# ebartrum/lightning_gan_zoo

Measured on AMD Instinct MI355X. Metric: images/sec (G+D step) at 64x64 bs=128/GPU, higher is better.
Workload: dtype f32; 1 GPU; dc_gan synthetic 64x64 bs=128/GPU, one optimizer cycle of 2 batches (Lightning alternation + toggle), reference optimizer, fp32; key=dc_gan_bs128, global_batch=128, parallelism=dp1, images_counted=2*bs*n_gpus per step (every batch of the cycle)

## Files before the change

include/gz_ops.h:

```cpp
#ifndef GZ_OPS_H
#define GZ_OPS_H

#include <stddef.h>

#ifdef __cplusplus
extern "C" {
#endif

#ifndef __HIP__
typedef struct ihipStream_t* hipStream_t;
#endif

#define GZ_ACT_NONE 0
#define GZ_ACT_RELU 1
#define GZ_ACT_LRELU 2
#define GZ_ACT_TANH 3


long long gz_conv2d_pack_fwd_elems(int K, int C, int KH, int KW);
long long gz_conv2d_pack_dgrad_elems(int K, int C, int KH, int KW, int S);

int gz_conv2d_pack_fwd(const float* w, float* wpack, int K, int C, int KH, int KW, hipStream_t stream);
int gz_conv2d_pack_dgrad(const float* w, float* wpack, int K, int C, int KH, int KW, int S, int P,
                         hipStream_t stream);
// ... 21 lines not shown

size_t gz_conv2d_wgrad_workspace_bytes(int N, int C, int H, int W, int K, int OH, int OW, int KH, int KW);
int gz_conv2d_wgrad_fuses_bias(int N, int C, int H, int W, int K, int OH, int OW, int KH, int KW, int S, int P);
int gz_conv2d_wgrad(const float* x, const float* y, float* dw, float* dbias, float* workspace, size_t ws_bytes, int N,
                    int C, int H, int W, int K, int OH, int OW, int KH, int KW, int S, int P, hipStream_t stream);

int gz_set_cu_budget(int cu_count);
int gz_get_cu_budget(void);

int gz_conv2d_plan(int op, int N, int C, int H, int W, int K, int OH, int OW, int KH, int KW, int S, int P, char* buf,
                   int buflen);

int gz_conv2d_wgrad_partial(const float* x, const float* y, float* dw, float* workspace, size_t ws_bytes, int N, int C,
                            int H, int W, int K, int OH, int OW, int KH, int KW, int S, int P, int* nz_out,
                            long long* stride_out, hipStream_t stream);
int gz_conv2d_wgrad_act_fuses(int N, int C, int H, int W, int K, int OH, int OW, int KH, int KW, int S, int P, int act);
int gz_conv2d_wgrad_act_partial(const float* x, const float* gy, const float* fwd_out, int act, float slope,
                                float* workspace, size_t ws_bytes, int N, int C, int H, int W, int K, int OH, int OW,
                                int KH, int KW, int S, int P, int* nz_out, long long* stride_out,
                                long long* bias_offset_out, hipStream_t stream);
int gz_conv2d_dgrad_act_fuses(int N, int C, int H, int W, int K, int OH, int OW, int KH, int KW, int S, int P, int act);
int gz_conv2d_dgrad_act(const float* gy, const float* fwd_out, int act, float slope, const float* wpack, float* x, int N,
                        int C, int H, int W, int K, int OH, int OW, int KH, int KW, int S, int P, hipStream_t stream);
int gz_reduce_multi_max_jobs(void);
int gz_reduce_multi_max_sources(void);
size_t gz_reduce_multi_table_bytes(void);
int gz_reduce_multi_add(void* table_host, float* out, long long count, int beta, const float* slabs, int nz,
                        long long stride);
int gz_reduce_multi(void* table_host, hipStream_t stream);

int gz_conv2d_fwd_stats_rows(int N, int C, int H, int W, int K, int OH, int OW, int KH, int KW, int S, int P);
int gz_conv2d_fwd_stats(const float* x, const float* wpack, float* y, float* stats, int N, int C, int H, int W, int K,
                        int OH, int OW, int KH, int KW, int S, int P, hipStream_t stream);
int gz_conv2d_dgrad_stats_rows(int N, int C, int H, int W, int K, int OH, int OW, int KH, int KW, int S, int P);
int gz_conv2d_fwd_stats_ws(const float* x, const float* wpack, float* y, float* stats, float* workspace, size_t ws_bytes,
                           int N, int C, int H, int W, int K, int OH, int OW, int KH, int KW, int S, int P,
                           hipStream_t stream);
int gz_conv2d_dgrad_stats_ws(const float* y, const float* wpack, float* x, float* stats, float* workspace,
                             size_t ws_bytes, int N, int C, int H, int W, int K, int OH, int OW, int KH, int KW, int S,
                             int P, hipStream_t stream);
int gz_conv2d_dgrad_stats(const float* y, const float* wpack, float* x, float* stats, int N, int C, int H, int W, int K,
                          int OH, int OW, int KH, int KW, int S, int P, hipStream_t stream);

int gz_conv2d_tile(int op, int N, int C, int H, int W, int K, int OH, int OW, int KH, int KW, int S);

int gz_gemm(const float* a, const float* b, const float* bias, float* c, float* workspace, size_t ws_bytes, int M,
// ... 247 lines not shown
```

lightning_gan_zoo_amd/core/models/standard_networks.py:

```python
import math
from collections import OrderedDict

import torch
from torch import nn

from ... import functional as F


class _GBlock(nn.Module):

    def __init__(self, cin, cout, stride, padding):
        super().__init__()
        self.transpose_conv = nn.ConvTranspose2d(cin, cout, 4, stride, padding, bias=False)
        self.batch_norm = nn.BatchNorm2d(cout)
        self.relu = nn.ReLU()
        self.stride, self.padding = stride, padding

    def forward(self, x):
        w = self.transpose_conv.weight
        bn = self.batch_norm
        F.ready(w, bn.weight, bn.bias)
        training = bn.training or bn.running_mean is None
        stats = None
        if self.stride == 1 and self.padding == 0 and x.shape[2] == 1 and x.shape[3] == 1:
            n = x.shape[0]
            y = F.matmul(x.reshape(n, -1), w.view(w.shape[0], -1), w).view(n, w.shape[1], 4, 4)
        elif self.stride == 2 and self.padding == 1:
            if training:
                y, stats = F.conv_transpose2d_with_stats(x, w, F.K4S2P1)
            else:
                y = F.conv_transpose2d(x, w, None, F.K4S2P1)
        else:
            raise RuntimeError("unsupported transposed-convolution geometry on the HIP path")
        return F.batch_norm_act(y, bn.weight, bn.bias, bn.running_mean, bn.running_var, bn.num_batches_tracked,
                                training, bn.momentum, bn.eps, F.ACT_RELU, 0.0, stats)


class _DBlock(nn.Module):

    def __init__(self, cin, cout, norm):
        super().__init__()
        self.conv = nn.Conv2d(cin, cout, 4, 2, 1, bias=False)
        if norm == "batch_norm":
            self.batch_norm = nn.BatchNorm2d(cout)
        elif norm == "instance_norm2d":
            self.instance_norm2d = nn.InstanceNorm2d(cout, affine=True)
        else:
            self.identity = nn.Identity()
        self.leaky_relu = nn.LeakyReLU(0.2)
        self.norm = norm

    def forward(self, x, groups=1):
        slope = self.leaky_relu.negative_slope
        F.ready(*self.parameters())
        if self.norm == "batch_norm":
            bn = self.batch_norm
# ... 33 lines not shown
    supports_stacked_batches = True
    gates_parameters = True

    def __init__(self, channels_img, features_d, norm="batch_norm", img_size=64, final_sigmoid=True):
        super().__init__()
        self.norm = norm
        n_blocks = int(math.log2(img_size // 8))
        blocks = [(f"block{i}", _DBlock(features_d * 2 ** (i - 1), features_d * 2 ** i, norm))
                  for i in range(1, n_blocks + 1)]
        conv_in = nn.Conv2d(channels_img, features_d, kernel_size=4, stride=2, padding=1, bias=False)
        conv_out = nn.Conv2d(features_d * 2 ** n_blocks, 1, kernel_size=4, stride=2, padding=0, bias=False)
        tail = ("sigmoid", nn.Sigmoid()) if final_sigmoid else ("identity", nn.Identity())
        self.disc = _DiscStack(OrderedDict(
            [("conv_in", conv_in), ("leaky_relu", nn.LeakyReLU(0.2))] + blocks + [("conv_out", conv_out), tail]))

    def forward(self, x, groups=1):
        if groups > 1 and self.norm == "batch_norm" and not self.training:
            raise RuntimeError("stacked batches with their own statistics exist in training mode only")
        return self.disc(x, groups)


class _GenStack(nn.Sequential):
    def forward(self, x):
        for name, m in self.named_children():
            if name.startswith("block"):
                x = m(x)
        F.ready(self.transpose_conv_out.weight)
        return F.conv_transpose2d(x, self.transpose_conv_out.weight, None, F.K4S2P1, F.ACT_TANH, 0.0)


class Generator(nn.Module):
    gates_parameters = True

    def __init__(self, channels_noise, channels_img, features_g, img_size=64):
        super().__init__()
        n_blocks = int(math.log2(img_size / 4))
        widths = [channels_noise] + [features_g * 2 ** (n_blocks - i) for i in range(n_blocks)]
        layers = [(f"block{i + 1}", _GBlock(widths[i], widths[i + 1], 1 if i == 0 else 2, 0 if i == 0 else 1))
                  for i in range(n_blocks)]
        layers.append(("transpose_conv_out", nn.ConvTranspose2d(features_g * 2, channels_img, kernel_size=4,
                                                                stride=2, padding=1, bias=False)))
        layers.append(("tanh", nn.Tanh()))
        self.net = _GenStack(OrderedDict(layers))

    def forward(self, x):
        return self.net(x.unsqueeze(-1).unsqueeze(-1))
```

lightning_gan_zoo_amd/csrc/gz_conv.hip:

```cpp
#include <cstdio>
#include <type_traits>

#include "gz_conv_choice.h"
#include "gz_conv_direct.h"
#include "gz_igemm.h"
#include "gz_reduce.h"
#include "../../include/gz_ops.h"

namespace gz {


static TileId pick_tile2(long long M, long long N, int ny, int kdim) {
    const bool off = knobs().no_igemm2;
    if (!off && N > 32 && N <= 64 && kdim >= 256) {
        const long long t = ((M + 511) / 512) * ny;
        if (t >= 2 * cus()) return T512x64;
        if (!knobs().no_tile64 && knobs().igemm2_tile == 0 && N == 64 && ((M + 255) / 256) * ny >= cus()) return T256x64;
        return T64x64;
    }
    if (off || N < 128 || kdim < 256) return T64x64;
    const long long t128 = ((M + 255) / 256) * ((N + 127) / 128) * ny;
    const long long t256 = ((M + 255) / 256) * ((N + 255) / 256) * ny;
    const int force = knobs().igemm2_tile;
    const int cu = cus();
// ... 948 lines not shown
        return run_gemm<Cfg, MContigLoader<Cfg::BM>, MContigLoader<Cfg::BN>>(a, b, bias, c, M, N, K, lda, ldb, ldc, act, slope, st, splits, slab);
    }
    if (!ta && tb) return run_gemm<Cfg, KContigLoader<Cfg::BM>, KContigLoader<Cfg::BN>>(a, b, bias, c, M, N, K, lda, ldb, ldc, act, slope, st, splits, slab);
    return run_gemm<Cfg, MContigLoader<Cfg::BM>, KContigLoader<Cfg::BN>>(a, b, bias, c, M, N, K, lda, ldb, ldc, act, slope, st, splits, slab);
}

}

using namespace gz;

typedef Geo<4, 4, 2, 1> G4421;
typedef Geo<5, 5, 2, 2> G5522;
typedef Geo<3, 3, 1, 1> G3311;
typedef Geo<1, 1, 1, 0> G1110;

#define GZ_GEOM_DISPATCH_OR(CALL, ELSE)                                 \
    if (KH == 4 && KW == 4 && S == 2 && P == 1) return CALL(G4421);     \
    if (KH == 5 && KW == 5 && S == 2 && P == 2) return CALL(G5522);     \
    if (KH == 3 && KW == 3 && S == 1 && P == 1) return CALL(G3311);     \
    if (KH == 1 && KW == 1 && S == 1 && P == 0) return CALL(G1110);     \
    return ELSE;
#define GZ_GEOM_DISPATCH(CALL) GZ_GEOM_DISPATCH_OR(CALL, GZ_ERR_UNSUPPORTED)

extern "C" {

size_t gz_conv2d_fwd_workspace_bytes(int N, int C, int H, int W, int K, int OH, int OW, int KH, int KW, int S, int P) {
    ConvShape s{N, C, H, W, K, OH, OW};
    if (!shape_ok(s, KH, KW, S, P)) return 0;
#define CALL(G) fwd_ws_bytes<G>(s)
    GZ_GEOM_DISPATCH_OR(CALL, 0)
#undef CALL
}

size_t gz_conv2d_dgrad_workspace_bytes(int N, int C, int H, int W, int K, int OH, int OW, int KH, int KW, int S,
                                       int P) {
    ConvShape s{N, C, H, W, K, OH, OW};
    if (!shape_ok(s, KH, KW, S, P)) return 0;
#define CALL(G) dgrad_ws_bytes<G>(s)
    GZ_GEOM_DISPATCH_OR(CALL, 0)
#undef CALL
}

int gz_conv2d_fwd(const float* x, const float* wpack, const float* bias, float* y, float* workspace, size_t ws_bytes,
                  int N, int C, int H, int W, int K, int OH, int OW, int KH, int KW, int S, int P, int act,
                  float slope, hipStream_t stream) {
    gz::clear_stale_error();
// ... 84 lines not shown
}

static bool dgrad_act_direct(const ConvShape& s, int KH, int KW, int S, int P, int act) {
    return KH == 4 && KW == 4 && S == 2 && P == 1 && (act == ACT_RELU || act == ACT_LRELU) && !knobs().no_act_fuse &&
           dgrad_direct<G4421>(s) && smallc_four_pos(s);
}

int gz_conv2d_dgrad_act_fuses(int N, int C, int H, int W, int K, int OH, int OW, int KH, int KW, int S, int P, int act) {
    ConvShape s{N, C, H, W, K, OH, OW};
    return shape_ok(s, KH, KW, S, P) && dgrad_act_direct(s, KH, KW, S, P, act) ? 1 : 0;
}

int gz_conv2d_dgrad_act(const float* gy, const float* fwd_out, int act, float slope, const float* wpack, float* x, int N,
                        int C, int H, int W, int K, int OH, int OW, int KH, int KW, int S, int P, hipStream_t stream) {
    gz::clear_stale_error();
    ConvShape s{N, C, H, W, K, OH, OW};
    if (!gy || !fwd_out || !wpack || !x || !shape_ok(s, KH, KW, S, P)) return GZ_ERR_BAD_SHAPE;
    if (too_large((long long)N * C * H * W) || too_large((long long)N * K * OH * OW)) return GZ_ERR_TOO_LARGE;
    if (!dgrad_act_direct(s, KH, KW, S, P, act) || (((uintptr_t)gy | (uintptr_t)x | (uintptr_t)fwd_out | (uintptr_t)wpack) & 15))
        return GZ_ERR_UNSUPPORTED;
    const float neg = act == ACT_RELU ? 0.f : slope;
    const int ks = smallc_split((long long)N * OH * OW / 4, K);
    return run_dgrad_smallc(gy, wpack, nullptr, x, s, ACT_NONE, 0.f, stream, ks, fwd_out, neg);
}

int gz_set_cu_budget(int cu_count) {
    if (cu_count <= 0) cu_count = 256;
    if (cu_count < 64) cu_count = 64;
    if (cu_count > 256) cu_count = 256;
    gz::cu_budget_ref().store(cu_count, std::memory_order_relaxed);
    return cu_count;
}

int gz_get_cu_budget(void) { return gz::cus(); }

static int stats_wm(TileId t) { return t == T128x32 ? 4 : 2; }
static int stats_tm_rows(TileId t, long long M) {
    if (t == T256x256 || t == T256x128) return (int)((M + 255) / 256) * 2;
    if (t == T512x64) return (int)((M + 511) / 512) * 4;
    if (t == T256x64) return (int)((M + 255) / 256) * 2;
    const int bm = t == T64x64 ? 64 : 128;
    return (int)((M + bm - 1) / bm) * stats_wm(t);
}

int gz_conv2d_fwd_stats_rows(int N, int C, int H, int W, int K, int OH, int OW, int KH, int KW, int S, int P) {
    ConvShape s{N, C, H, W, K, OH, OW};
// ... 225 lines not shown
```

lightning_gan_zoo_amd/csrc/gz_conv_direct.h:

```cpp
#pragma once
#include "gz_conv_choice.h"

namespace gz {

bool smallc_four_pos(const ConvShape& s);
bool dgrad_direct5_ok(const ConvShape& s);
int smallc_split(long long M4, int K);
int run_dgrad_smallc(const float* y, const float* wp, const float* bias, float* x, const ConvShape& s, int act, float slope,
                     hipStream_t st, int ks, const float* mask = nullptr, float mask_neg = 0.f);
int run_dgrad_smallc5(const float* y, const float* wp, const float* bias, float* x, const ConvShape& s, int act, float slope,
                      hipStream_t st, int ks);

bool conv3_fewk_ok(int CI, int CO, int H, int W);
bool conv3_smallch_ok(int N, int CI, int CO, int H, int W);
int run_conv3_smallch(const float* in, const float* wp, const float* bias, float* out, int N, int CI, int CO, int H, int W,
                      int tap_major, int flip, int act, float slope, hipStream_t st, Loader ld);

bool wgrad_fewk_ok(const ConvShape& s);
bool wgrad_smallch_ok(const ConvShape& s, int KH, int KW, int S, int P);
int wgrad_smallch_blocks(const ConvShape& s);
int run_wgrad_smallch(const float* x, const float* y, float* dw, float* dbias, float* ws, size_t ws_bytes, const ConvShape& s,
                      Loader ld, hipStream_t st);

bool wgrad_k4s2p1_fewc_ok(const ConvShape& s);
int wgrad_k4s2p1_fewc_blocks(const ConvShape& s);
int run_wgrad_k4s2p1_fewc(const float* x, const float* y, const float* fwd_out, int act, float slope, float* dw, float* ws,
                          size_t ws_bytes, const ConvShape& s, hipStream_t st);

}
```

lightning_gan_zoo_amd/csrc/gz_conv_direct.hip:

```cpp
#include "gz_conv_direct.h"
#include "gz_knobs.h"
#include "gz_pack_layout.h"
#include "gz_reduce.h"
#include "../../include/gz_ops.h"

namespace gz {

template <int C>
__global__ __launch_bounds__(256) void dgrad_smallc_k4s2p1_kernel(const float* __restrict__ y,
                                                                  const float* __restrict__ wp,
                                                                  const float* __restrict__ bias,
                                                                  float* __restrict__ x, ConvShape s,
                                                                  FastDiv div_ohw, FastDiv div_ow, int act,
                                                                  float slope) {
    const int OHW = s.OH * s.OW;
    const uint32_t M = (uint32_t)s.N * OHW;
    const uint32_t m = blockIdx.x * 256u + threadIdx.x;
    const bool m_ok = m < M;
    const uint32_t n = fdiv(m, div_ohw);
    const uint32_t pix = m - n * (uint32_t)OHW;
    const int a = (int)fdiv(pix, div_ow);
    const int b = (int)(pix - (uint32_t)a * (uint32_t)s.OW);
    __amdgpu_buffer_rsrc_t rsrc = make_rsrc(y, (uint32_t)s.N * s.K * OHW * 4u);
    uint32_t voff[3][3];
// ... 31 lines not shown
                    for (int tx = 0; tx < 2; ++tx) {
                        const float yv = v[(py + 1) / 2 - ty + 1][(px + 1) / 2 - tx + 1];
                        const f32x4 w4 = *reinterpret_cast<const f32x4*>(wrow + (ty * 2 + tx) * 4);
#pragma unroll
                        for (int c = 0; c < C; ++c) acc[py][px][c] = fmaf(yv, w4[c], acc[py][px][c]);
                    }
            }
    }
    if (!m_ok) return;
#pragma unroll
    for (int c = 0; c < C; ++c) {
        const float bv = bias ? bias[c] : 0.f;
#pragma unroll
        for (int py = 0; py < 2; ++py) {
            f32x2 o;
            o.x = act_fwd(acc[py][0][c] + bv, act, slope);
            o.y = act_fwd(acc[py][1][c] + bv, act, slope);
            float* dst = x + (((long long)n * C + c) * s.H + (2 * a + py)) * s.W + 2 * b;
            *reinterpret_cast<f32x2*>(dst) = o;
        }
    }
}

template <int C, int KS, int KH = 4>
__global__ __launch_bounds__(KS > 4 ? 64 * KS : 256) void dgrad_smallc4_k4s2p1_kernel(const float* __restrict__ y,
                                                                   const float* __restrict__ wp,
                                                                   const float* __restrict__ bias,
                                                                   float* __restrict__ x, ConvShape s,
                                                                   FastDiv div_ohw4, FastDiv div_ow4, int act,
                                                                   float slope, const float* __restrict__ mask = nullptr,
                                                                   float mask_neg = 0.f) {
    constexpr int P = KH == 4 ? 1 : 2, TMAX = (KH + 1) / 2;
    __shared__ float part[KS > 1 ? KS / 2 : 1][KS > 1 ? 16 * C : 1][64];
    const int OW4 = s.OW >> 2, OHW = s.OH * s.OW;
    const uint32_t M4 = (uint32_t)s.N * s.OH * OW4;
    const int lane = threadIdx.x & 63, wave = KS > 1 ? __builtin_amdgcn_readfirstlane(threadIdx.x >> 6) : 0;
    const uint32_t m = KS > 1 ? blockIdx.x * 64u + lane : blockIdx.x * 256u + threadIdx.x;
    const bool m_ok = m < M4;
    const uint32_t n = fdiv(m, div_ohw4);
    const uint32_t pix = m - n * (uint32_t)(s.OH * OW4);
    const int a = (int)fdiv(pix, div_ow4);
    const int b = (int)(pix - (uint32_t)a * (uint32_t)OW4) * 4;
    __amdgpu_buffer_rsrc_t rsrc = make_rsrc(y, (uint32_t)s.N * s.K * OHW * 4u);
    uint32_t voff[3];
#pragma unroll
    for (int dy = 0; dy < 3; ++dy) {
        int oy = a + dy - 1;
        bool ok = m_ok && (unsigned)oy < (unsigned)s.OH;
        voff[dy] = ok ? (n * (uint32_t)(s.K * OHW) + (uint32_t)(oy * s.OW + b)) * 4u : OOB;
    }
    const bool has_l = b > 0, has_r = b + 4 < s.OW;
    float acc[4][2][2][C];
#pragma unroll
    for (int q = 0; q < 4; ++q)
#pragma unroll
        for (int i = 0; i < 2; ++i)
#pragma unroll
            for (int j = 0; j < 2; ++j)
#pragma unroll
                for (int c = 0; c < C; ++c) acc[q][i][j][c] = 0.f;
    const int kpad = round_bk(s.K);
    const long long phase_stride = KH == 4 ? (long long)s.K * 16
                                           : (long long)TMAX * TMAX * kpad * 4;
    const __amdgpu_buffer_rsrc_t rmask = make_rsrc(mask ? mask : y, (uint32_t)s.N * s.K * OHW * 4u);
    f32x4 nxt[3], mnx[3];
    if constexpr (KS > 1) {
#pragma unroll
        for (int dy = 0; dy < 3; ++dy) {
            nxt[dy] = bload4(rsrc, wave < s.K ? voff[dy] : OOB, (uint32_t)wave * (uint32_t)OHW * 4u);
            if (mask) mnx[dy] = bload4(rmask, wave < s.K ? voff[dy] : OOB, (uint32_t)wave * (uint32_t)OHW * 4u);
        }
// ... 5 lines not shown
            const bool more = ko + KS < s.K;
            const uint32_t soff = (uint32_t)(more ? ko + KS : ko) * (uint32_t)OHW * 4u;
#pragma unroll
            for (int dy = 0; dy < 3; ++dy) {
                cur[dy] = nxt[dy];
                nxt[dy] = bload4(rsrc, more ? voff[dy] : OOB, soff);
                if (mask) {
                    mcur[dy] = mnx[dy];
                    mnx[dy] = bload4(rmask, more ? voff[dy] : OOB, soff);
                }
            }
        } else {
#pragma unroll
            for (int dy = 0; dy < 3; ++dy) {
                cur[dy] = bload4(rsrc, voff[dy], (uint32_t)ko * (uint32_t)OHW * 4u);
                if (mask) mcur[dy] = bload4(rmask, voff[dy], (uint32_t)ko * (uint32_t)OHW * 4u);
            }
        }
        if (mask) {
#pragma unroll
            for (int dy = 0; dy < 3; ++dy)
#pragma unroll
                for (int e = 0; e < 4; ++e) cur[dy][e] = mcur[dy][e] > 0.f ? cur[dy][e] : cur[dy][e] * mask_neg;
        }
#pragma unroll
        for (int dy = 0; dy < 3; ++dy) {
            const f32x4 r = cur[dy];
            const float l = __shfl_up(r.w, 1), rr = __shfl_down(r.x, 1);
            v[dy][0] = has_l ? l : 0.f;
            v[dy][1] = r.x; v[dy][2] = r.y; v[dy][3] = r.z; v[dy][4] = r.w;
            v[dy][5] = has_r ? rr : 0.f;
        }
#pragma unroll
        for (int py = 0; py < 2; ++py)
#pragma unroll
            for (int px = 0; px < 2; ++px) {
                const int ny = dg_taps(KH, 2, P, py), nx = dg_taps(KH, 2, P, px);
                const float* wrow = KH == 4 ? wp + (py * 2 + px) * phase_stride + (long long)ko * 16
                                            : wp + (py * 2 + px) * phase_stride + (long long)ko * 4;
#pragma unroll
                for (int ty = 0; ty < TMAX; ++ty)
#pragma unroll
                    for (int tx = 0; tx < TMAX; ++tx) {
                        if (ty < ny && tx < nx) {
                            const f32x4 w4 = *reinterpret_cast<const f32x4*>(
                                KH == 4 ? wrow + (ty * 2 + tx) * 4 : wrow + (long long)(ty * nx + tx) * kpad * 4);
// ... 130 lines not shown
        else if (ks == 4)
            hipLaunchKernelGGL((dgrad_smallc4_k4s2p1_kernel<C, 4>), dim3((unsigned)((M4 + 63) / 64)), dim3(256), 0, st, y,
                               wp, bias, x, s, make_fastdiv(s.OH * (s.OW / 4)), make_fastdiv(s.OW / 4), act, slope, mask,
                               mask_neg);
        else
            hipLaunchKernelGGL((dgrad_smallc4_k4s2p1_kernel<C, 1>), dim3((unsigned)((M4 + 255) / 256)), dim3(256), 0, st,
                               y, wp, bias, x, s, make_fastdiv(s.OH * (s.OW / 4)), make_fastdiv(s.OW / 4), act, slope, mask,
                               mask_neg);
        return launch_status();
    }
    if (mask) return GZ_ERR_UNSUPPORTED;
    hipLaunchKernelGGL(dgrad_smallc_k4s2p1_kernel<C>, dim3((unsigned)((M + 255) / 256)), dim3(256), 0, st, y, wp, bias,
                       x, s, make_fastdiv(s.OH * s.OW), make_fastdiv(s.OW), act, slope);
    return launch_status();
}

int run_dgrad_smallc(const float* y, const float* wp, const float* bias, float* x, const ConvShape& s, int act, float slope,
                     hipStream_t st, int ks, const float* mask, float mask_neg) {
    switch (s.C) {
        case 1: return run_dgrad_smallc_c<1>(y, wp, bias, x, s, act, slope, st, ks, mask, mask_neg);
        case 2: return run_dgrad_smallc_c<2>(y, wp, bias, x, s, act, slope, st, ks, mask, mask_neg);
        case 3: return run_dgrad_smallc_c<3>(y, wp, bias, x, s, act, slope, st, ks, mask, mask_neg);
        default: return run_dgrad_smallc_c<4>(y, wp, bias, x, s, act, slope, st, ks, mask, mask_neg);
    }
}

int run_dgrad_smallc5(const float* y, const float* wp, const float* bias, float* x, const ConvShape& s, int act, float slope,
                      hipStream_t st, int ks) {
    switch (s.C) {
        case 1: return run_dgrad_smallc5_c<1>(y, wp, bias, x, s, act, slope, st, ks);
        case 2: return run_dgrad_smallc5_c<2>(y, wp, bias, x, s, act, slope, st, ks);
        case 3: return run_dgrad_smallc5_c<3>(y, wp, bias, x, s, act, slope, st, ks);
        default: return run_dgrad_smallc5_c<4>(y, wp, bias, x, s, act, slope, st, ks);
    }
}

template <int OT, int IT>
__global__ __launch_bounds__(256) void conv3x3_smallch_kernel(const float* __restrict__ in, const float* __restrict__ wp,
                                                              const float* __restrict__ bias, float* __restrict__ out,
                                                              int N, int CI, int CO, int H, int W, int groups,
                                                              FastDiv div_seg, FastDiv div_h, int tap_major, int inpad,
                                                              int ld, int flip, int act, float slope) {
    constexpr int CB = IT * 4;
    __shared__ float Ws[9 * CB * OT * 64];
    for (int e = threadIdx.x; e < 9 * CB * OT * 64; e += 256) {
        const int i = e & 15, q = (e >> 4) & 3;
// ... 652 lines not shown
```

lightning_gan_zoo_amd/csrc/gz_igemm_loaders.h:

```cpp
#pragma once
#include "gz_common.h"
#include "gz_knobs.h"
#include "gz_pack_layout.h"
#include <type_traits>

namespace gz {

constexpr int NT = 256;

#ifndef GZ_IGEMM_NO_DMA
#define GZ_IGEMM_DMA 1
#else
#define GZ_IGEMM_DMA 0
#endif
__device__ __forceinline__ void bload_lds4(__amdgpu_buffer_rsrc_t r, float* lds_wave_base, uint32_t voff,
                                           uint32_t soff) {
    __builtin_amdgcn_raw_ptr_buffer_load_lds(r, (__attribute__((address_space(3))) void*)lds_wave_base, 4, voff, soff, 0,
                                             0);
}
__device__ __forceinline__ void bload_lds16(__amdgpu_buffer_rsrc_t r, float* lds_wave_base, uint32_t voff,
                                            uint32_t soff) {
    __builtin_amdgcn_raw_ptr_buffer_load_lds(r, (__attribute__((address_space(3))) void*)lds_wave_base, 16, voff, soff,
                                             0, 0);
}
// ... 670 lines not shown
        rsrc = make_rsrc(p.y, (uint32_t)s.N * s.K * s.OH * s.OW * 4u);
        kl = tid & 15;
        m_l = tid >> 4;
        OHW = s.OH * s.OW; OW = s.OW; KOHW = s.K * OHW;
        div_ohw = p.g.div_ohw; div_ow = p.g.div_ow;
        const int dy = kl / p.g.CW, dx = kl % p.g.CW;
#pragma unroll
        for (int j = 0; j < EPT; ++j) {
            int ko = tile * BM + m_l + 16 * j;
            voff[j] = ko < s.K ? (uint32_t)(ko * OHW + dy * OW + dx) * 4u : OOB;
        }
    }
    __device__ __forceinline__ void issue(int kc) {
        uint32_t p0 = (uint32_t)kc * BK;
        uint32_t n = fdiv(p0, div_ohw);
        uint32_t rem = p0 - n * (uint32_t)OHW;
        uint32_t soff = (n * (uint32_t)KOHW + rem) * 4u;
#pragma unroll
        for (int j = 0; j < EPT; ++j) r[j] = bload(rsrc, voff[j], soff);
    }
    __device__ __forceinline__ void commit(float* dst) const {
#pragma unroll
        for (int j = 0; j < EPT; ++j) dst[kl * LD + m_l + 16 * j] = r[j];
    }
};

template <int BN, int KH, int KW, int S, int P>
struct WgBLoaderRow : LoaderDefaults {
    struct Params {
        const float* x;
        ConvShape s;
        WgRowGeom g;
        int KTOT, NTOT;
    };
    static constexpr int LD = BN + 2;
    static constexpr int NPARTS = 0;
    __device__ __forceinline__ void issue_lds_part(int, float*, int) {}
    static constexpr bool DMA = false;
    __device__ __forceinline__ void issue_lds(int, float*) {}
    static constexpr int EPT = BN / 16;
    __amdgpu_buffer_rsrc_t rsrc;
    uint32_t voff[EPT];
    uint32_t flags[EPT];
    int kl, n_l, OHW, OW, OH, W, CHW, CW, R;
    FastDiv div_ohw, div_ow;
    float r[EPT];
// ... 504 lines not shown
```

lightning_gan_zoo_amd/functional/_base.py:

```python
import ctypes
import os
import weakref
from collections import namedtuple

import torch

from .._lib import check, lib

ACT_NONE, ACT_RELU, ACT_LRELU, ACT_TANH = 0, 1, 2, 3

Geom = namedtuple("Geom", "kh kw stride pad")
K4S2P1 = Geom(4, 4, 2, 1)


def _p(t):
    return None if t is None else ctypes.c_void_p(t.data_ptr())


_raw_stream = getattr(torch._C, "_cuda_getCurrentRawStream", None)


def _stream():
    if _raw_stream is not None:
        return ctypes.c_void_p(_raw_stream(torch.cuda.current_device()))
# ... 407 lines not shown
def _sink_conv_wgrad(w, x, g, geom):
    if not _sinks.enabled or not isinstance(w, torch.nn.Parameter) or (w.numel() & 3):
        return False
    if w.grad is not None and (w.grad.data_ptr() & 15 or not w.grad.is_contiguous() or w.grad.dtype != torch.float32):
        return False
    N, C, H, W = x.shape
    _, K, OH, OW = g.shape
    nbytes = lib.gz_conv2d_wgrad_workspace_bytes(N, C, H, W, K, OH, OW, geom.kh, geom.kw)
    if not nbytes:
        return False
    if id(w) in _sinks.deferred:
        _sinks.deferred_jobs.append((w, x, g, geom))
        return True
    ws = _ws(nbytes // 4, x.device)
    dw = torch.empty((K, C, geom.kh, geom.kw), device=x.device, dtype=torch.float32)
    nz, stride = ctypes.c_int(0), ctypes.c_longlong(0)
    _timed(2, (N, C, H, W, K, OH, OW), geom, 2.0 * N * OH * OW * K * C * geom.kh * geom.kw, lambda: check(
        lib.gz_conv2d_wgrad_partial(_p(x), _p(g), _p(dw), _p(ws), nbytes, N, C, H, W, K, OH, OW, geom.kh, geom.kw,
                                    geom.stride, geom.pad, ctypes.byref(nz), ctypes.byref(stride), _stream()),
        "conv2d_wgrad_partial"))
    src = (ws, nz.value, stride.value) if nz.value > 1 else (dw, 1, w.numel())
    if src[2] & 3:
        return False if nz.value <= 1 else _sink_fail("slab stride")
    _sinks.pending.setdefault(id(w), [w, []])[1].append(src)
    return True


def _sink_conv_wgrad_act(w, b, x, g, y, geom, act, slope):
    if not _sinks.enabled or act not in (ACT_RELU, ACT_LRELU) or id(w) in _sinks.deferred:
        return False
    for p_ in (w, b):
        if p_ is None:
            continue
        if not isinstance(p_, torch.nn.Parameter) or (p_.numel() & 3):
            return False
        if p_.grad is not None and (p_.grad.data_ptr() & 15 or not p_.grad.is_contiguous() or p_.grad.dtype != torch.float32):
            return False
    N, C, H, W = x.shape
    _, K, OH, OW = g.shape
    shape = (N, C, H, W, K, OH, OW, geom.kh, geom.kw, geom.stride, geom.pad)
    if not lib.gz_conv2d_wgrad_act_fuses(*shape, act):
        return False
    g, y = _req(g), _req(y)
    nbytes = lib.gz_conv2d_wgrad_workspace_bytes(N, C, H, W, K, OH, OW, geom.kh, geom.kw)
    ws = _ws(nbytes // 4, x.device)
    nz, stride, boff = ctypes.c_int(0), ctypes.c_longlong(0), ctypes.c_longlong(0)
# ... 147 lines not shown
```

lightning_gan_zoo_amd/functional/_norm.py:

```python
import ctypes
import os
import weakref
from collections import namedtuple

import torch

from .._lib import check, lib
from ._base import *
from ._conv import *

def _norm_ws(x, N, C):
    return _ws(max(lib.gz_norm_workspace_bytes(N, C) // 4, 1), x.device)


def _sink_small_pair(a, b):
    if not _sinks.enabled:
        return None
    for p in (a, b):
        if not isinstance(p, torch.nn.Parameter) or not p.requires_grad:
            return None
    if (a.grad is None) != (b.grad is None):
        return None
    if a.grad is None:
        a.grad = torch.empty_like(a, memory_format=torch.contiguous_format)
        b.grad = torch.empty_like(b, memory_format=torch.contiguous_format)
        return a.grad, b.grad, 0
    for p in (a, b):
        if not p.grad.is_contiguous() or p.grad.dtype != torch.float32:
            return None
    return a.grad, b.grad, 1


class _BatchNormAct(torch.autograd.Function):

    @staticmethod
    def forward(ctx, x, gamma, beta, running_mean, running_var, nbt, training, momentum, eps, act, slope, stats=None,
                groups=1):
        x = _req(x, "x")
        N, C = x.shape[:2]
        inner = x.numel() // (N * C)
        if groups > 1 and (not training or N % groups):
            raise RuntimeError("statistics groups need training mode and a batch that is a multiple of the group count")
        coef = torch.empty(4 * groups * C, device=x.device, dtype=torch.float32)
        st = _stream()
        if training and not _NORM_UNFUSED:
            out = torch.empty_like(x)
            fused = stats is not None and stats.numel()
            ws = None if fused else _norm_ws(x, N, C)
            check(lib.gz_batchnorm_act_fwd_fused(_p(x), _p(stats) if fused else None, stats.shape[0] if fused else 0,
                                                 (N // groups) * inner if fused else 0, _p(gamma), _p(beta), _p(coef),
                                                 _p(running_mean), _p(running_var), _p(nbt), _p(ws), _p(out), N, C, inner,
                                                 eps, momentum, groups, act, slope, st), "batchnorm_act_fwd_fused")
            ctx.save_for_backward(x, coef, gamma, beta)
# ... 18 lines not shown

    @staticmethod
    @torch.autograd.function.once_differentiable
    def backward(ctx, gout):
        x, coef, gamma, beta = ctx.saved_tensors
        N, C, inner, act, slope, training, groups = ctx.cfg
        gout = _req(gout)
        nones = (None,) * 10
        if not training:
            st = _stream()
            gp = gout
            if act != ACT_NONE:
                out = torch.empty_like(x)
                check(lib.gz_norm_act_fwd(_p(x), _p(coef), _p(out), N, C, inner, 1, act, slope, st), "norm_act_fwd")
                gp = _act_bwd_raw(gout, out, act, slope)
            scale, mean, rstd = coef[:C], coef[2 * C:3 * C], coef[3 * C:]
            dx = None
            if ctx.needs_input_grad[0]:
                dx = _rowscale_raw(gp.view(N * C, inner), scale.repeat(N).contiguous(), N * C, inner, False).view_as(x)
            dbeta = _channel_sum_raw(gp)
            sgx = _rowdot_raw(gp.view(N * C, inner), x.view(N * C, inner), False).view(N, C).sum(0)
            dgamma = rstd * (sgx - mean * dbeta)
            return (dx, dgamma if ctx.needs_input_grad[1] else None, dbeta if ctx.needs_input_grad[2] else None) + nones
        need_dx = ctx.needs_input_grad[0]
        dx = torch.empty_like(x) if need_dx else None
        sunk = _sink_small_pair(gamma, beta) if (ctx.needs_input_grad[1] and ctx.needs_input_grad[2]) else None
        if sunk is not None:
            dgamma, dbeta, accumulate = sunk
        else:
            dgamma = torch.empty(C, device=x.device, dtype=torch.float32)
            dbeta = torch.empty(C, device=x.device, dtype=torch.float32)
            accumulate = 0
        kbuf = torch.empty(2 * groups * C, device=x.device, dtype=torch.float32)
        ws = _norm_ws(x, N, C)
        check(lib.gz_batchnorm_act_bwd_g(_p(gout), _p(x), _p(coef), _p(dx), _p(dgamma), _p(dbeta), _p(ws), _p(kbuf), N,
                                         C, inner, act, slope, groups, accumulate, _stream()), "norm_act_bwd")
        if sunk is not None:
            return (dx, None, None) + nones
        return (dx, dgamma if ctx.needs_input_grad[1] else None, dbeta if ctx.needs_input_grad[2] else None) + nones


def batch_norm_act(x, gamma, beta, running_mean, running_var, nbt, training, momentum=0.1, eps=1e-5,
                   act=ACT_NONE, slope=0.0, stats=None, groups=1):
    if groups > 1 and stats is not None and stats.numel():
        rows, M = stats.shape[0], x.shape[0] * (x.numel() // (x.shape[0] * x.shape[1]))
        if rows % groups or M % rows or (M // groups) % (M // rows):
            stats = None
    return _BatchNormAct.apply(x, gamma, beta, running_mean, running_var, nbt, training, momentum, eps, act, slope,
                               stats, groups)


class _RowNormAct(torch.autograd.Function):

    @staticmethod
    def forward(ctx, x, gamma, beta, eps, act, slope):
        x = _req(x, "x")
        N, C = x.shape[:2]
        inner = x.numel() // (N * C)
        coef = torch.empty(4 * N * C, device=x.device, dtype=torch.float32)
        out = torch.empty_like(x)
        check(lib.gz_rownorm_act_fwd(_p(x), _p(gamma), _p(beta), _p(coef), _p(out), N, C, inner, eps, 0, 0, act, slope,
                                     _stream()), "rownorm_act_fwd")
        ctx.save_for_backward(x, gamma, coef, beta)
        ctx.cfg = (N, C, inner, act, slope)
        return out

    @staticmethod
    def backward(ctx, gout):
        x, gamma, coef, beta = ctx.saved_tensors
        if (not torch.is_grad_enabled() and gamma is not None and ctx.needs_input_grad[1] and ctx.needs_input_grad[2]):
            sunk = _sink_small_pair(gamma, beta)
            if sunk is not None:
# ... 61 lines not shown
```

Before: 46490 images/s.

## Fuse generator's last BatchNorm+ReLU into the output transposed-conv kernels

```diff
diff --git a/include/gz_ops.h b/include/gz_ops.h
--- a/include/gz_ops.h
+++ b/include/gz_ops.h
@@ -67,6 +67,15 @@
 int gz_conv2d_dgrad_act_fuses(int N, int C, int H, int W, int K, int OH, int OW, int KH, int KW, int S, int P, int act);
 int gz_conv2d_dgrad_act(const float* gy, const float* fwd_out, int act, float slope, const float* wpack, float* x, int N,
                         int C, int H, int W, int K, int OH, int OW, int KH, int KW, int S, int P, hipStream_t stream);
+int gz_conv2d_dgrad_norm_fuses(int N, int C, int H, int W, int K, int OH, int OW, int KH, int KW, int S, int P, int norm_act);
+int gz_conv2d_dgrad_norm(const float* yraw, const float* coef, int norm_act, float norm_slope, const float* wpack, float* x,
+                         int N, int C, int H, int W, int K, int OH, int OW, int KH, int KW, int S, int P, int act,
+                         float slope, hipStream_t stream);
+int gz_conv2d_wgrad_norm_fuses(int N, int C, int H, int W, int K, int OH, int OW, int KH, int KW, int S, int P, int norm_act);
+int gz_conv2d_wgrad_norm_partial(const float* x, const float* yraw, const float* coef, int norm_act, float norm_slope,
+                                 float* dw, float* workspace, size_t ws_bytes, int N, int C, int H, int W, int K, int OH,
+                                 int OW, int KH, int KW, int S, int P, int* nz_out, long long* stride_out,
+                                 hipStream_t stream);
 int gz_reduce_multi_max_jobs(void);
 int gz_reduce_multi_max_sources(void);
 size_t gz_reduce_multi_table_bytes(void);
diff --git a/lightning_gan_zoo_amd/core/models/standard_networks.py b/lightning_gan_zoo_amd/core/models/standard_networks.py
--- a/lightning_gan_zoo_amd/core/models/standard_networks.py
+++ b/lightning_gan_zoo_amd/core/models/standard_networks.py
@@ -17,6 +17,9 @@
         self.stride, self.padding = stride, padding
 
     def forward(self, x):
+        return self.norm(*self.conv(x))
+
+    def conv(self, x):
         w = self.transpose_conv.weight
         bn = self.batch_norm
         F.ready(w, bn.weight, bn.bias)
@@ -32,6 +35,10 @@
                 y = F.conv_transpose2d(x, w, None, F.K4S2P1)
         else:
             raise RuntimeError("unsupported transposed-convolution geometry on the HIP path")
+        return y, stats, training
+
+    def norm(self, y, stats, training):
+        bn = self.batch_norm
         return F.batch_norm_act(y, bn.weight, bn.bias, bn.running_mean, bn.running_var, bn.num_batches_tracked,
                                 training, bn.momentum, bn.eps, F.ACT_RELU, 0.0, stats)
 
@@ -111,11 +118,26 @@
 
 class _GenStack(nn.Sequential):
     def forward(self, x):
-        for name, m in self.named_children():
-            if name.startswith("block"):
-                x = m(x)
-        F.ready(self.transpose_conv_out.weight)
-        return F.conv_transpose2d(x, self.transpose_conv_out.weight, None, F.K4S2P1, F.ACT_TANH, 0.0)
+        blocks = [m for name, m in self.named_children() if name.startswith("block")]
+        w_out = self.transpose_conv_out.weight
+        last = blocks[-1] if blocks and not (blocks[-1]._forward_hooks or blocks[-1]._forward_pre_hooks) else None
+        for m in (blocks[:-1] if last is not None else blocks):
+            x = m(x)
+        if last is not None:
+            y, stats, training = last.conv(x)
+            F.ready(w_out)
+            bn = last.batch_norm
+            out = None
+            if training and last.stride == 2:
+                out = F.batch_norm_act_conv_transpose2d(y, bn.weight, bn.bias, bn.running_mean, bn.running_var,
+                                                        bn.num_batches_tracked, training, bn.momentum, bn.eps, F.ACT_RELU,
+                                                        0.0, stats, w_out, F.K4S2P1, F.ACT_TANH)
+            if out is not None:
+                return out
+            x = last.norm(y, stats, training)
+        else:
+            F.ready(w_out)
+        return F.conv_transpose2d(x, w_out, None, F.K4S2P1, F.ACT_TANH, 0.0)
 
 
 class Generator(nn.Module):
diff --git a/lightning_gan_zoo_amd/csrc/gz_conv.hip b/lightning_gan_zoo_amd/csrc/gz_conv.hip
--- a/lightning_gan_zoo_amd/csrc/gz_conv.hip
+++ b/lightning_gan_zoo_amd/csrc/gz_conv.hip
@@ -994,6 +994,21 @@
     return ELSE;
 #define GZ_GEOM_DISPATCH(CALL) GZ_GEOM_DISPATCH_OR(CALL, GZ_ERR_UNSUPPORTED)
 
+template <class Cfg>
+static int run_wgrad_norm(const float* x, const float* yraw, const float* coef, int nact, float nslope, float* dw, float* ws,
+                          const ConvShape& s, const Choice& c, hipStream_t st) {
+    using G = G4421;
+    const int KTOT = s.N * s.OH * s.OW;
+    const int NTOT = s.C * G::kh * G::kw;
+    WgRowGeom rg;
+    wg_row_geom<G>(s, &rg);
+    using AL = WgALoaderRowNorm<Cfg::BM>;
+    using BL = WgBLoaderRow<Cfg::BN, G::kh, G::kw, G::s, G::p>;
+    typename AL::Params pa{yraw, s, rg, KTOT, coef, nact, nslope};
+    typename BL::Params pb{x, s, rg, KTOT, NTOT};
+    return launch_wgrad_igemm<G, Cfg, AL, BL>(pa, pb, dw, ws, s, KTOT, NTOT, c, st);
+}
+
 extern "C" {
 
 size_t gz_conv2d_fwd_workspace_bytes(int N, int C, int H, int W, int K, int OH, int OW, int KH, int KW, int S, int P) {
@@ -1124,6 +1139,65 @@
     const float neg = act == ACT_RELU ? 0.f : slope;
     const int ks = smallc_split((long long)N * OH * OW / 4, K);
     return run_dgrad_smallc(gy, wpack, nullptr, x, s, ACT_NONE, 0.f, stream, ks, fwd_out, neg);
+}
+
+static bool dgrad_norm_direct(const ConvShape& s, int KH, int KW, int S, int P, int nact) {
+    return KH == 4 && KW == 4 && S == 2 && P == 1 && nact == ACT_RELU && !knobs().no_act_fuse && dgrad_direct<G4421>(s) &&
+           smallc_four_pos(s);
+}
+
+int gz_conv2d_dgrad_norm_fuses(int N, int C, int H, int W, int K, int OH, int OW, int KH, int KW, int S, int P, int norm_act) {
+    ConvShape s{N, C, H, W, K, OH, OW};
+    return shape_ok(s, KH, KW, S, P) && dgrad_norm_direct(s, KH, KW, S, P, norm_act) ? 1 : 0;
+}
+
+int gz_conv2d_dgrad_norm(const float* yraw, const float* coef, int norm_act, float norm_slope, const float* wpack, float* x,
+                         int N, int C, int H, int W, int K, int OH, int OW, int KH, int KW, int S, int P, int act,
+                         float slope, hipStream_t stream) {
+    gz::clear_stale_error();
+    ConvShape s{N, C, H, W, K, OH, OW};
+    if (!yraw || !coef || !wpack || !x || !shape_ok(s, KH, KW, S, P)) return GZ_ERR_BAD_SHAPE;
+    if (too_large((long long)N * C * H * W) || too_large((long long)N * K * OH * OW)) return GZ_ERR_TOO_LARGE;
+    if (!dgrad_norm_direct(s, KH, KW, S, P, norm_act) || (((uintptr_t)yraw | (uintptr_t)x | (uintptr_t)wpack) & 15))
+        return GZ_ERR_UNSUPPORTED;
+    const int ks = smallc_split((long long)N * OH * OW / 4, K);
+    return run_dgrad_smallc_norm(yraw, coef, norm_act, norm_slope, wpack, x, s, act, slope, stream, ks);
+}
+
+static bool wgrad_norm_igemm(const Choice& c, int nact) {
+    return c.kind == KIgemm && c.loader == LWgRow && (c.tile == T128x64 || c.tile == T64x64) &&
+           (nact == ACT_NONE || nact == ACT_RELU || nact == ACT_LRELU) && !knobs().no_act_fuse;
+}
+
+int gz_conv2d_wgrad_norm_fuses(int N, int C, int H, int W, int K, int OH, int OW, int KH, int KW, int S, int P, int norm_act) {
+    ConvShape s{N, C, H, W, K, OH, OW};
+    if (!shape_ok(s, KH, KW, S, P) || !(KH == 4 && KW == 4 && S == 2 && P == 1) || C > 4) return 0;
+    return wgrad_norm_igemm(choose_wgrad<G4421>(s, kIdeal), norm_act) ? 1 : 0;
+}
+
+int gz_conv2d_wgrad_norm_partial(const float* x, const float* yraw, const float* coef, int norm_act, float norm_slope,
+                                 float* dw, float* workspace, size_t ws_bytes, int N, int C, int H, int W, int K, int OH,
+                                 int OW, int KH, int KW, int S, int P, int* nz_out, long long* stride_out,
+                                 hipStream_t stream) {
+    gz::clear_stale_error();
+    if (!nz_out || !stride_out || !x || !yraw || !coef || !dw) return GZ_ERR_BAD_SHAPE;
+    ConvShape s{N, C, H, W, K, OH, OW};
+    if (!shape_ok(s, KH, KW, S, P)) return GZ_ERR_BAD_SHAPE;
+    if (too_large((long long)N * C * H * W) || too_large((long long)N * K * OH * OW)) return GZ_ERR_TOO_LARGE;
+    if (!(KH == 4 && KW == 4 && S == 2 && P == 1) || C > 4) return GZ_ERR_UNSUPPORTED;
+    *nz_out = 1;
+    *stride_out = (long long)K * C * KH * KW;
+    const Facts f = facts_of((const void*)((uintptr_t)x | (uintptr_t)yraw), dw, workspace, ws_bytes, false, false);
+    const Choice c = choose_wgrad<G4421>(s, f);
+    if (!wgrad_norm_igemm(c, norm_act)) return GZ_ERR_UNSUPPORTED;
+    WgDefer d{1, *stride_out};
+    tl_wg_defer = &d;
+    const int rc = c.tile == T128x64 ? run_wgrad_norm<Cfg128x64>(x, yraw, coef, norm_act, norm_slope, dw, workspace, s, c, stream)
+                                     : run_wgrad_norm<Cfg64x64>(x, yraw, coef, norm_act, norm_slope, dw, workspace, s, c, stream);
+    tl_wg_defer = nullptr;
+    *nz_out = d.nz;
+    *stride_out = d.stride;
+    return rc;
 }
 
 int gz_set_cu_budget(int cu_count) {
diff --git a/lightning_gan_zoo_amd/csrc/gz_conv_direct.h b/lightning_gan_zoo_amd/csrc/gz_conv_direct.h
--- a/lightning_gan_zoo_amd/csrc/gz_conv_direct.h
+++ b/lightning_gan_zoo_amd/csrc/gz_conv_direct.h
@@ -8,6 +8,8 @@
 int smallc_split(long long M4, int K);
 int run_dgrad_smallc(const float* y, const float* wp, const float* bias, float* x, const ConvShape& s, int act, float slope,
                      hipStream_t st, int ks, const float* mask = nullptr, float mask_neg = 0.f);
+int run_dgrad_smallc_norm(const float* y, const float* coef, int nact, float nslope, const float* wp, float* x,
+                          const ConvShape& s, int act, float slope, hipStream_t st, int ks);
 int run_dgrad_smallc5(const float* y, const float* wp, const float* bias, float* x, const ConvShape& s, int act, float slope,
                       hipStream_t st, int ks);
 
diff --git a/lightning_gan_zoo_amd/csrc/gz_conv_direct.hip b/lightning_gan_zoo_amd/csrc/gz_conv_direct.hip
--- a/lightning_gan_zoo_amd/csrc/gz_conv_direct.hip
+++ b/lightning_gan_zoo_amd/csrc/gz_conv_direct.hip
@@ -77,7 +77,7 @@
     }
 }
 
-template <int C, int KS, int KH = 4>
+template <int C, int KS, int KH = 4, int NORM = -1>
 __global__ __launch_bounds__(KS > 4 ? 64 * KS : 256) void dgrad_smallc4_k4s2p1_kernel(const float* __restrict__ y,
                                                                    const float* __restrict__ wp,
                                                                    const float* __restrict__ bias,
@@ -85,6 +85,8 @@
                                                                    FastDiv div_ohw4, FastDiv div_ow4, int act,
                                                                    float slope, const float* __restrict__ mask = nullptr,
                                                                    float mask_neg = 0.f) {
+    [[maybe_unused]] const float* const coef = mask;
+    if constexpr (NORM >= 0) mask = nullptr;
     constexpr int P = KH == 4 ? 1 : 2, TMAX = (KH + 1) / 2;
     __shared__ float part[KS > 1 ? KS / 2 : 1][KS > 1 ? 16 * C : 1][64];
     const int OW4 = s.OW >> 2, OHW = s.OH * s.OW;
@@ -98,10 +100,12 @@
     const int b = (int)(pix - (uint32_t)a * (uint32_t)OW4) * 4;
     __amdgpu_buffer_rsrc_t rsrc = make_rsrc(y, (uint32_t)s.N * s.K * OHW * 4u);
     uint32_t voff[3];
+    bool row_ok[3];
 #pragma unroll
     for (int dy = 0; dy < 3; ++dy) {
         int oy = a + dy - 1;
         bool ok = m_ok && (unsigned)oy < (unsigned)s.OH;
+        row_ok[dy] = ok;
         voff[dy] = ok ? (n * (uint32_t)(s.K * OHW) + (uint32_t)(oy * s.OW + b)) * 4u : OOB;
     }
     const bool has_l = b > 0, has_r = b + 4 < s.OW;
@@ -153,6 +157,14 @@
             for (int dy = 0; dy < 3; ++dy)
 #pragma unroll
                 for (int e = 0; e < 4; ++e) cur[dy][e] = mcur[dy][e] > 0.f ? cur[dy][e] : cur[dy][e] * mask_neg;
+        }
+        if constexpr (NORM >= 0) {
+            const float sc = coef[ko], sh = coef[s.K + ko];
+#pragma unroll
+            for (int dy = 0; dy < 3; ++dy)
+#pragma unroll
+                for (int e = 0; e < 4; ++e)
+                    cur[dy][e] = row_ok[dy] ? act_fwd(__builtin_fmaf(cur[dy][e], sc, sh), NORM, mask_neg) : 0.f;
         }
 #pragma unroll
         for (int dy = 0; dy < 3; ++dy) {
@@ -329,6 +341,36 @@
         case 2: return run_dgrad_smallc_c<2>(y, wp, bias, x, s, act, slope, st, ks, mask, mask_neg);
         case 3: return run_dgrad_smallc_c<3>(y, wp, bias, x, s, act, slope, st, ks, mask, mask_neg);
         default: return run_dgrad_smallc_c<4>(y, wp, bias, x, s, act, slope, st, ks, mask, mask_neg);
+    }
+}
+
+template <int C>
+static int run_dgrad_smallc_norm_c(const float* y, const float* coef, int nact, float nslope, const float* wp, float* x,
+                                   const ConvShape& s, int act, float slope, hipStream_t st, int ks) {
+    if (nact != ACT_RELU) return GZ_ERR_UNSUPPORTED;
+    const long long M4 = (long long)s.N * s.OH * s.OW / 4;
+    const FastDiv d_ohw4 = make_fastdiv(s.OH * (s.OW / 4)), d_ow4 = make_fastdiv(s.OW / 4);
+    if (ks == 8)
+        hipLaunchKernelGGL((dgrad_smallc4_k4s2p1_kernel<C, 8, 4, ACT_RELU>), dim3((unsigned)((M4 + 63) / 64)), dim3(512), 0,
+                           st, y, wp, (const float*)nullptr, x, s, d_ohw4, d_ow4, act, slope, coef, 0.f);
+    else if (ks == 4)
+        hipLaunchKernelGGL((dgrad_smallc4_k4s2p1_kernel<C, 4, 4, ACT_RELU>), dim3((unsigned)((M4 + 63) / 64)), dim3(256), 0,
+                           st, y, wp, (const float*)nullptr, x, s, d_ohw4, d_ow4, act, slope, coef, 0.f);
+    else if (ks == 1)
+        hipLaunchKernelGGL((dgrad_smallc4_k4s2p1_kernel<C, 1, 4, ACT_RELU>), dim3((unsigned)((M4 + 255) / 256)), dim3(256), 0,
+                           st, y, wp, (const float*)nullptr, x, s, d_ohw4, d_ow4, act, slope, coef, 0.f);
+    else
+        return GZ_ERR_UNSUPPORTED;
+    return launch_status();
+}
+
+int run_dgrad_smallc_norm(const float* y, const float* coef, int nact, float nslope, const float* wp, float* x,
+                          const ConvShape& s, int act, float slope, hipStream_t st, int ks) {
+    switch (s.C) {
+        case 1: return run_dgrad_smallc_norm_c<1>(y, coef, nact, nslope, wp, x, s, act, slope, st, ks);
+        case 2: return run_dgrad_smallc_norm_c<2>(y, coef, nact, nslope, wp, x, s, act, slope, st, ks);
+        case 3: return run_dgrad_smallc_norm_c<3>(y, coef, nact, nslope, wp, x, s, act, slope, st, ks);
+        default: return run_dgrad_smallc_norm_c<4>(y, coef, nact, nslope, wp, x, s, act, slope, st, ks);
     }
 }
 
diff --git a/lightning_gan_zoo_amd/csrc/gz_igemm_loaders.h b/lightning_gan_zoo_amd/csrc/gz_igemm_loaders.h
--- a/lightning_gan_zoo_amd/csrc/gz_igemm_loaders.h
+++ b/lightning_gan_zoo_amd/csrc/gz_igemm_loaders.h
@@ -716,6 +716,40 @@
     __device__ __forceinline__ void commit(float* dst) const {
 #pragma unroll
         for (int j = 0; j < EPT; ++j) dst[kl * LD + m_l + 16 * j] = r[j];
+    }
+};
+
+template <int BM>
+struct WgALoaderRowNorm : WgALoaderRow<BM> {
+    using Base = WgALoaderRow<BM>;
+    struct Params {
+        const float* y;
+        ConvShape s;
+        WgRowGeom g;
+        int KTOT;
+        const float* coef;
+        int act;
+        float slope;
+    };
+    float sc[Base::EPT], sh[Base::EPT];
+    int act;
+    float slope;
+    __device__ __forceinline__ void init(const Params& p, int tile, int y, int tid) {
+        Base::init(typename Base::Params{p.y, p.s, p.g, p.KTOT}, tile, y, tid);
+        act = p.act;
+        slope = p.slope;
+#pragma unroll
+        for (int j = 0; j < Base::EPT; ++j) {
+            const int ko = tile * BM + this->m_l + 16 * j;
+            const bool ok = ko < p.s.K;
+            sc[j] = ok ? p.coef[ko] : 0.f;
+            sh[j] = ok ? p.coef[p.s.K + ko] : 0.f;
+        }
+    }
+    __device__ __forceinline__ void commit(float* dst) const {
+#pragma unroll
+        for (int j = 0; j < Base::EPT; ++j)
+            dst[this->kl * Base::LD + this->m_l + 16 * j] = act_fwd(__builtin_fmaf(this->r[j], sc[j], sh[j]), act, slope);
     }
 };
 
diff --git a/lightning_gan_zoo_amd/functional/_base.py b/lightning_gan_zoo_amd/functional/_base.py
--- a/lightning_gan_zoo_amd/functional/_base.py
+++ b/lightning_gan_zoo_amd/functional/_base.py
@@ -453,6 +453,49 @@
     src = (ws, nz.value, stride.value) if nz.value > 1 else (dw, 1, w.numel())
     if src[2] & 3:
         return False if nz.value <= 1 else _sink_fail("slab stride")
+    _sinks.pending.setdefault(id(w), [w, []])[1].append(src)
+    return True
+
+
+def _conv_dgrad_norm_raw(yraw, coef, nact, nslope, w, geom, hw, act, slope):
+    N, K, OH, OW = yraw.shape
+    C = w.shape[1]
+    H, W = hw
+    shape = (N, C, H, W, K, OH, OW, geom.kh, geom.kw, geom.stride, geom.pad)
+    if not lib.gz_conv2d_dgrad_norm_fuses(*shape, nact):
+        return None
+    wp = _packed(w, "d", geom)
+    x = torch.empty((N, C, H, W), device=yraw.device, dtype=torch.float32)
+    if (yraw.data_ptr() | x.data_ptr() | wp.data_ptr()) & 15:
+        return None
+    _timed(1, (N, C, H, W, K, OH, OW), geom, 2.0 * N * OH * OW * K * C * geom.kh * geom.kw, lambda: check(
+        lib.gz_conv2d_dgrad_norm(_p(yraw), _p(coef), nact, float(nslope), _p(wp), _p(x), *shape, act, float(slope),
+                                 _stream()), "conv2d_dgrad_norm"))
+    return x
+
+
+def _sink_conv_wgrad_norm(w, x, yraw, coef, nact, nslope, geom):
+    if not _sinks.enabled or not isinstance(w, torch.nn.Parameter) or (w.numel() & 3) or id(w) in _sinks.deferred:
+        return False
+    if w.grad is not None and (w.grad.data_ptr() & 15 or not w.grad.is_contiguous() or w.grad.dtype != torch.float32):
+        return False
+    N, C, H, W = x.shape
+    _, K, OH, OW = yraw.shape
+    shape = (N, C, H, W, K, OH, OW, geom.kh, geom.kw, geom.stride, geom.pad)
+    if not lib.gz_conv2d_wgrad_norm_fuses(*shape, nact):
+        return False
+    nbytes = lib.gz_conv2d_wgrad_workspace_bytes(N, C, H, W, K, OH, OW, geom.kh, geom.kw)
+    if not nbytes:
+        return False
+    ws = _ws(nbytes // 4, x.device)
+    dw = torch.empty((K, C, geom.kh, geom.kw), device=x.device, dtype=torch.float32)
+    nz, stride = ctypes.c_int(0), ctypes.c_longlong(0)
+    _timed(2, (N, C, H, W, K, OH, OW), geom, 2.0 * N * OH * OW * K * C * geom.kh * geom.kw, lambda: check(
+        lib.gz_conv2d_wgrad_norm_partial(_p(x), _p(yraw), _p(coef), nact, float(nslope), _p(dw), _p(ws), nbytes, *shape,
+                                         ctypes.byref(nz), ctypes.byref(stride), _stream()), "conv2d_wgrad_norm_partial"))
+    src = (ws, nz.value, stride.value) if nz.value > 1 else (dw, 1, w.numel())
+    if src[2] & 3:
+        _sink_fail("slab stride")
     _sinks.pending.setdefault(id(w), [w, []])[1].append(src)
     return True
 
diff --git a/lightning_gan_zoo_amd/functional/_norm.py b/lightning_gan_zoo_amd/functional/_norm.py
--- a/lightning_gan_zoo_amd/functional/_norm.py
+++ b/lightning_gan_zoo_amd/functional/_norm.py
@@ -29,6 +29,25 @@
         if not p.grad.is_contiguous() or p.grad.dtype != torch.float32:
             return None
     return a.grad, b.grad, 1
+
+
+def _bn_train_bwd(gout, x, coef, gamma, beta, cfg, needs):
+    N, C, inner, act, slope, _, groups = cfg
+    dx = torch.empty_like(x) if needs[0] else None
+    sunk = _sink_small_pair(gamma, beta) if (needs[1] and needs[2]) else None
+    if sunk is not None:
+        dgamma, dbeta, accumulate = sunk
+    else:
+        dgamma = torch.empty(C, device=x.device, dtype=torch.float32)
+        dbeta = torch.empty(C, device=x.device, dtype=torch.float32)
+        accumulate = 0
+    kbuf = torch.empty(2 * groups * C, device=x.device, dtype=torch.float32)
+    ws = _norm_ws(x, N, C)
+    check(lib.gz_batchnorm_act_bwd_g(_p(gout), _p(x), _p(coef), _p(dx), _p(dgamma), _p(dbeta), _p(ws), _p(kbuf), N,
+                                     C, inner, act, slope, groups, accumulate, _stream()), "norm_act_bwd")
+    if sunk is not None:
+        return (dx, None, None)
+    return (dx, dgamma if needs[1] else None, dbeta if needs[2] else None)
 
 
 class _BatchNormAct(torch.autograd.Function):
@@ -93,22 +112,7 @@
             sgx = _rowdot_raw(gp.view(N * C, inner), x.view(N * C, inner), False).view(N, C).sum(0)
             dgamma = rstd * (sgx - mean * dbeta)
             return (dx, dgamma if ctx.needs_input_grad[1] else None, dbeta if ctx.needs_input_grad[2] else None) + nones
-        need_dx = ctx.needs_input_grad[0]
-        dx = torch.empty_like(x) if need_dx else None
-        sunk = _sink_small_pair(gamma, beta) if (ctx.needs_input_grad[1] and ctx.needs_input_grad[2]) else None
-        if sunk is not None:
-            dgamma, dbeta, accumulate = sunk
-        else:
-            dgamma = torch.empty(C, device=x.device, dtype=torch.float32)
-            dbeta = torch.empty(C, device=x.device, dtype=torch.float32)
-            accumulate = 0
-        kbuf = torch.empty(2 * groups * C, device=x.device, dtype=torch.float32)
-        ws = _norm_ws(x, N, C)
-        check(lib.gz_batchnorm_act_bwd_g(_p(gout), _p(x), _p(coef), _p(dx), _p(dgamma), _p(dbeta), _p(ws), _p(kbuf), N,
-                                         C, inner, act, slope, groups, accumulate, _stream()), "norm_act_bwd")
-        if sunk is not None:
-            return (dx, None, None) + nones
-        return (dx, dgamma if ctx.needs_input_grad[1] else None, dbeta if ctx.needs_input_grad[2] else None) + nones
+        return _bn_train_bwd(gout, x, coef, gamma, beta, ctx.cfg, ctx.needs_input_grad[:3]) + nones
 
 
 def batch_norm_act(x, gamma, beta, running_mean, running_var, nbt, training, momentum=0.1, eps=1e-5,
@@ -119,6 +123,72 @@
             stats = None
     return _BatchNormAct.apply(x, gamma, beta, running_mean, running_var, nbt, training, momentum, eps, act, slope,
                                stats, groups)
+
+
+_NO_EDGE_FUSE = bool(os.environ.get("GZ_NO_EDGE_FUSE"))
+
+
+class _BatchNormActConvT(torch.autograd.Function):
+
+    @staticmethod
+    def forward(ctx, x, gamma, beta, running_mean, running_var, nbt, momentum, eps, act, slope, stats, w, geom, hw,
+                out_act):
+        N, C = x.shape[:2]
+        inner = x.numel() // (N * C)
+        coef = torch.empty(4 * C, device=x.device, dtype=torch.float32)
+        check(lib.gz_batchnorm_finalize_g(_p(stats), stats.shape[0], N * inner, _p(gamma), _p(beta), _p(coef),
+                                          _p(running_mean), _p(running_var), _p(nbt), C, eps, momentum, 1, _stream()),
+              "batchnorm_finalize")
+        img = _conv_dgrad_norm_raw(x, coef, act, slope, w, geom, hw, out_act, 0.0)
+        if img is None:
+            raise RuntimeError("lightning_gan_zoo_amd: the fused output layer was chosen for a shape it does not take")
+        ctx.save_for_backward(x, coef, gamma, beta, w, img)
+        ctx.cfg = (N, C, inner, act, slope, True, 1)
+        ctx.geom, ctx.out_act = geom, out_act
+        return img
+
+    @staticmethod
+    @torch.autograd.function.once_differentiable
+    def backward(ctx, v):
+        x, coef, gamma, beta, w, img = ctx.saved_tensors
+        N, C, inner, act, slope = ctx.cfg[:5]
+        geom = ctx.geom
+        v = _req(v)
+        if ctx.out_act != ACT_NONE:
+            v = _act_bwd_raw(v, img, ctx.out_act, 0.0)
+        needs = ctx.needs_input_grad
+        gy = _conv_fwd_raw(v, w, None, geom, ACT_NONE, 0.0) if any(needs[:3]) else None
+        dw = None
+        if needs[11] and not _sink_conv_wgrad_norm(w, v, x, coef, act, slope, geom):
+            y = torch.empty_like(x)
+            check(lib.gz_norm_act_fwd_g(_p(x), _p(coef), _p(y), N, C, inner, 1, 1, act, slope, _stream()), "norm_act_fwd")
+            if not _sink_conv_wgrad(w, v, y, geom):
+                dw = _conv_wgrad_raw(v, y, geom)
+        dx = dgamma = dbeta = None
+        if gy is not None:
+            dx, dgamma, dbeta = _bn_train_bwd(gy, x, coef, gamma, beta, ctx.cfg, needs[:3])
+        return (dx, dgamma, dbeta) + (None,) * 8 + (dw, None, None, None)
+
+
+def batch_norm_act_conv_transpose2d(x, gamma, beta, running_mean, running_var, nbt, training, momentum, eps, act, slope,
+                                    stats, w, geom=K4S2P1, out_act=ACT_NONE):
+    from .. import functional as _pkg
+    if _pkg.batch_norm_act is not batch_norm_act or _pkg.conv_transpose2d is not conv_transpose2d:
+        return None
+    if (_NO_EDGE_FUSE or _NORM_UNFUSED or not training or not _sinks.enabled or stats is None or not stats.numel()
+            or not x.is_cuda or x.dtype != torch.float32 or not x.is_contiguous() or not w.is_contiguous()
+            or x.dim() != 4 or running_mean is None):
+        return None
+    N, K, OH, OW = x.shape
+    C = w.shape[1]
+    H, W = (OH - 1) * geom.stride - 2 * geom.pad + geom.kh, (OW - 1) * geom.stride - 2 * geom.pad + geom.kw
+    shape = (N, C, H, W, K, OH, OW, geom.kh, geom.kw, geom.stride, geom.pad)
+    if w.shape[0] != K or not lib.gz_conv2d_dgrad_norm_fuses(*shape, act) or not lib.gz_conv2d_wgrad_norm_fuses(*shape, act):
+        return None
+    if (x.data_ptr() | _packed(w, "d", geom).data_ptr()) & 15:
+        return None
+    return _BatchNormActConvT.apply(x, gamma, beta, running_mean, running_var, nbt, momentum, eps, act, slope, stats, w,
+                                    geom, (H, W), out_act)
 
 
 class _RowNormAct(torch.autograd.Function):
```

Result: no change. 46890 images/s (median of 6 runs) (+0.9%).
